# VisualComputingInstitute/diffusion-e2e-ft

Hardware: AMD Instinct MI355X
Metric: images/sec (768x768, 1-step UNet fwd) full path: VAE encode + SD-v2 UNet @t=999 + VAE decode (higher is better)
Workload: dtype f16

## Files before the change

### diffusion-e2e-ft_amd/_lib.py

```python
import ctypes as C
import os

import torch

from . import build as _build

_LIB = None

F32, F16, BF16 = 0, 1, 2
_DT = {torch.float32: F32, torch.float16: F16, torch.bfloat16: BF16}


def dtype_id(dt):
    try:
        return _DT[dt]
    except KeyError:
        raise TypeError("libe2eft supports float32/float16/bfloat16, got %s" % dt)


class ConvDesc(C.Structure):
    _fields_ = [(n, C.c_int32) for n in (
        "dtype", "batch", "hin", "win", "hl", "wl", "c1", "ldx1", "c2", "ldx2", "kh", "kw", "stride", "pad_t", "pad_l",
        "hout", "wout", "cout", "ldo", "ldr", "ldw")] + [("alpha", C.c_float)]

# ... 14 lines not shown
                                          "ldo")] + [("scale", C.c_float)]


class NormalEvalDesc(C.Structure):
    _fields_ = [(n, C.c_int32) for n in ("batch", "height", "width", "reserved")] + [
        ("pred_stride", C.c_int64 * 4), ("gt_stride", C.c_int64 * 4), ("mask_stride", C.c_int64 * 3)]


class D2ntDesc(C.Structure):
    _fields_ = [(n, C.c_int32) for n in ("batch", "height", "width", "refine", "out_format")] + [("depth_scale", C.c_float)]


D2NT_F32, D2NT_U16, D2NT_U8 = range(3)


class HypersimDesc(C.Structure):
    _fields_ = [(n, C.c_int32) for n in ("batch", "height", "width", "color_dtype", "distance_dtype", "depth_format")] + [
        ("focal", C.c_double), ("scale_numerator", C.c_double)]


HYPERSIM_DEPTH_U16, HYPERSIM_DEPTH_F32 = range(2)
HYPERSIM_RECORD = 16


class DepthGtDesc(C.Structure):
    _fields_ = ([(n, C.c_int32) for n in ("batch", "h0", "w0", "raw_dtype")] + [("divisor", C.c_double)]
                + [(n, C.c_int32) for n in ("inf_to_zero", "crop_top", "crop_left", "crop_h", "crop_w")] + [("min_depth", C.c_float), ("max_depth", C.c_float)]
                + [(n, C.c_int32) for n in ("win_y0", "win_y1", "win_x0", "win_x1", "use_ext_mask")])


GT_U16, GT_I32, GT_F32 = range(3)


OPT_PERSISTENT, OPT_PERSISTENT_GRID, OPT_NARROW_CONV, OPT_NARROW_MFMA, OPT_IGEMM_GENERAL_OPERANDS, OPT_IGEMM2_WAVES, OPT_PATCH_CONV, OPT_THIN_INPUT_CONV, OPT_FUSED_NORM, OPT_ATTN_DMA, OPT_UPCONV_PHASES, OPT_PATCH_CONV_2X2, OPT_PERSISTENT_MIN_QROUNDS, OPT_GN_APPLY_ITERS, OPT_F32_SPLIT = range(15)

_P = C.c_void_p
_I = C.c_int32
_L = C.c_int64
_F = C.c_float
_Z = C.c_size_t

SIGNATURES = {
    "e2eft_version": (_I, []),
    "e2eft_last_error": (C.c_char_p, []),
    "e2eft_build_id": (C.c_char_p, []),
    "e2eft_set_option": (_I, [_I, _I]),
    "e2eft_get_option": (_I, [_I]),
    "e2eft_conv2d_fwd": (_I, [C.POINTER(ConvDesc), _P, _P, _P, _P, _P, _P, _P, _P]),
    "e2eft_gemm": (_I, [C.POINTER(GemmDesc), _P, _P, _P, _P, _P, _P]),
    "e2eft_conv2d_fwd_gnstats": (_I, [C.POINTER(ConvDesc), _P, _P, _P, _P, _P, _P, _P, _P, _Z, C.POINTER(C.c_int32), _P]),
    "e2eft_conv2d_splitk_workspace_bytes": (_Z, [C.POINTER(ConvDesc)]),
    "e2eft_conv2d_fwd_splitk": (_I, [C.POINTER(ConvDesc), _P, _P, _P, _P, _P, _P, _P, _P, _Z, _P]),
    "e2eft_gemm_gnstats": (_I, [C.POINTER(GemmDesc), _P, _P, _P, _P, _P, _I, _P, _Z, C.POINTER(C.c_int32), _P]),
    "e2eft_groupnorm_fwd_pre": (_I, [C.POINTER(GroupNormDesc), _P, _P, _P, _P, _P, _P, _I, _P, _I, _P, _Z, _P]),
    "e2eft_groupnorm_coeff_offset": (_Z, [C.POINTER(GroupNormDesc)]),
    "e2eft_groupnorm_fwd_stats": (_I, [C.POINTER(GroupNormDesc), _P, _P, _P, _P, _I, _P, _I, _P, _Z, _P]),
    "e2eft_conv2d_fwd_normed_supported": (_I, [C.POINTER(ConvDesc)]),
    "e2eft_upconv2x_fwd_supported": (_I, [C.POINTER(ConvDesc)]),
    "e2eft_upconv2x_fwd": (_I, [C.POINTER(ConvDesc), _P, _P, _P, _P, _P, _Z, C.POINTER(C.c_int32), _P]),
    "e2eft_groupnorm_fwd_split": (_I, [C.POINTER(GroupNormDesc), _P, _P, _P, _P, _I, _P, _P, _I, _P, _Z, _P]),
    "e2eft_f32_split_weight": (_I, [_P, _L, _I, _P, _P, _P]),
    "e2eft_f32_split2_cat": (_I, [_P, _I, _I, _P, _I, _I, _L, _P, _I, _P, _P]),
    "e2eft_f32_split2": (_I, [_P, _L, _I, _I, _P, _I, _P, _P]),
    "e2eft_conv2d_fwd_f32split_supported": (_I, [C.POINTER(ConvDesc)]),
    "e2eft_conv2d_fwd_f32split": (_I, [C.POINTER(ConvDesc), _P, _P, _P, _P, _P, _P, _P, _P, _Z, C.POINTER(C.c_int32), _P]),
    "e2eft_upconv2x_fwd_f32split_supported": (_I, [C.POINTER(ConvDesc)]),
    "e2eft_upconv2x_fwd_f32split": (_I, [C.POINTER(ConvDesc), _P, _P, _P, _P, _P, _P, _P, _Z, C.POINTER(C.c_int32), _P]),
    "e2eft_gemm_f32split_supported": (_I, [C.POINTER(GemmDesc)]),
    "e2eft_gemm_f32split": (_I, [C.POINTER(GemmDesc), _P, _P, _P, _P, _P, _P, _P, _P]),
    "e2eft_conv2d_fwd_normed": (_I, [C.POINTER(ConvDesc), _P, _P, _P, _I, _P, _P, _P, _P, _P, _P, _Z, C.POINTER(C.c_int32), _P]),
    "e2eft_groupnorm_workspace_bytes": (_Z, [C.POINTER(GroupNormDesc)]),
    "e2eft_groupnorm_fwd": (_I, [C.POINTER(GroupNormDesc), _P, _P, _P, _P, _P, _P, _Z, _P]),
    "e2eft_layernorm_fwd": (_I, [_I, _L, _I, _I, _I, _F, _P, _P, _P, _P, _P]),
    "e2eft_geglu_fwd": (_I, [_I, _L, _I, _I, _I, _P, _P, _P]),
    "e2eft_softmax_rows": (_I, [_I, _L, _I, _L, _F, _P, _P]),
    "e2eft_softmax_rows_causal": (_I, [_I, _L, _I, _L, _F, _I, _P, _P]),
    "e2eft_attn_fwd": (_I, [C.POINTER(AttnDesc), _P, _P, _P, _P, _P]),
    "e2eft_attn_fwd_lse": (_I, [C.POINTER(AttnDesc), _P, _P, _P, _P, _P, _P]),
    "e2eft_attn512_workspace_bytes": (_Z, [C.POINTER(AttnDesc)]),
    "e2eft_attn512_fwd": (_I, [C.POINTER(AttnDesc), _P, _P, _P, _P, _P, _Z, _P]),
    "e2eft_attn_bwd_workspace_bytes": (_Z, [C.POINTER(AttnDesc)]),
    "e2eft_attn_bwd": (_I, [C.POINTER(AttnDesc), _P, _P, _P, _P, _P, _I, _P, _P, _I, _P, _I, _P, _I, _P, _Z, _P]),
    "e2eft_nchw_to_nhwc": (_I, [_I, _I, _I, _I, _I, _I, _I, _F, _F, _P, _P, _P]),
    "e2eft_nhwc_to_nchw": (_I, [_I, _I, _I, _I, _I, _I, _F, _F, _P, _P, _P]),
    "e2eft_copy_scale": (_I, [_I, _L, _I, _I, _I, _F, _F, _P, _P, _P]),
    "e2eft_add": (_I, [_I, _L, _I, _I, _I, _I, _P, _P, _P, _P]),
    "e2eft_timestep_embedding": (_I, [_I, _I, _I, _P, _P, _P]),
    "e2eft_silu": (_I, [_I, _L, _P, _P, _P]),
    "e2eft_depth_head": (_I, [_I, _I, _L, _I, _I, _P, _P, _P]),
    "e2eft_normal_head": (_I, [_I, _I, _I, _I, _I, _I, _F, _P, _P, _P]),
    "e2eft_ssi_loss_workspace_bytes": (_Z, [_I]),
    "e2eft_ssi_loss_fwd": (_I, [_I, _I, _P, _P, _P, _P, _P, _P, _Z, _P]),
    "e2eft_angular_loss_workspace_bytes": (_Z, [_I]),
    "e2eft_angular_loss_fwd": (_I, [_I, _I, _P, _P, _P, _P, _P, _Z, _P]),
    "e2eft_conv2d_dgrad": (_I, [C.POINTER(ConvDesc), _P, _I, _I, _P, _I, _P, _I, _P]),
    "e2eft_conv2d_wgrad_workspace_bytes": (_Z, [C.POINTER(ConvDesc), _I]),
    "e2eft_conv2d_wgrad": (_I, [C.POINTER(ConvDesc), _P, _I, _P, _P, _P, _Z, C.POINTER(C.c_int32), _P]),
    "e2eft_conv2d_im2col_t": (_I, [C.POINTER(ConvDesc), _P, _P, _P, _L, _P]),
    "e2eft_transpose": (_I, [_I, _I, _L, _I, _L, _L, _L, _L, _L, _P, _P, _P]),
    "e2eft_colsum_workspace_bytes": (_Z, [_I, _L, _I]),
    "e2eft_colsum": (_I, [_I, _I, _L, _I, _L, _F, _P, _P, _P, _Z, _P]),
    "e2eft_upsample_nearest_bwd": (_I, [_I, _I, _I, _I, _I, _I, _I, _I, _I, _P, _P, _P]),
    "e2eft_groupnorm_bwd_workspace_bytes": (_Z, [C.POINTER(GroupNormDesc)]),
    "e2eft_groupnorm_bwd": (_I, [C.POINTER(GroupNormDesc), _P, _P, _P, _P, _P, _I, _P, _I, _P, _P, _P, _P, _Z, _P]),
    "e2eft_groupnorm_bwd_add": (_I, [C.POINTER(GroupNormDesc), _P, _P, _P, _P, _P, _I, _P, _I, _P, _I, _P, _P, _P, _P, _Z, _P]),
    "e2eft_layernorm_bwd_workspace_bytes": (_Z, [_L, _I]),
# ... 107 lines not shown
```

### diffusion-e2e-ft_amd/csrc/api.hip

```cpp
#include "common.h"
#include <atomic>

namespace e2eft {

static thread_local char g_err[512] = "";

char* err_buf() { return g_err; }

int fail(int code, const char* fmt, ...) {
    va_list ap;
    va_start(ap, fmt);
    vsnprintf(g_err, sizeof(g_err), fmt, ap);
    va_end(ap);
    return code;
}

int check_launch(const char* what) {
    hipError_t e = hipGetLastError();
    if (e != hipSuccess) return fail(E2EFT_ERR_LAUNCH, "%s: launch failed: %s", what, hipGetErrorString(e));
    return E2EFT_OK;
}

static std::atomic<int> g_cus_of_device[64];
int device_cus() {
    int dev = 0;
    if (hipGetDevice(&dev) != hipSuccess || dev < 0 || dev >= 64) return 0;
    int n = g_cus_of_device[dev].load(std::memory_order_relaxed);
    if (n == 0) {
        if (hipDeviceGetAttribute(&n, hipDeviceAttributeMultiprocessorCount, dev) != hipSuccess || n < 8) return 0;
        n &= ~7;
        g_cus_of_device[dev].store(n, std::memory_order_relaxed);
    }
    return n;
}

static thread_local char g_tag[96] = "";
void tag_kernel(const char* fmt, ...) {
    va_list ap;
    va_start(ap, fmt);
    vsnprintf(g_tag, sizeof(g_tag), fmt, ap);
    va_end(ap);
}
const char* last_tag() { return g_tag; }

static std::atomic<int> g_opt[E2EFT_OPT_COUNT] = {{1}, {0}, {1}, {1}, {0}, {0}, {1}, {1}, {1}, {1}, {1}, {1}, {2}, {0}, {1}};

int option(int key) { return g_opt[key].load(std::memory_order_relaxed); }

}

extern "C" int e2eft_set_option(int32_t key, int32_t value) {
    using namespace e2eft;
    E2EFT_REQUIRE(key >= 0 && key < E2EFT_OPT_COUNT, "set_option: unknown key %d", key);
    bool ok = value == 0 || value == 1;
    if (key == E2EFT_OPT_PERSISTENT_GRID) ok = value == 0 || (value >= 8 && value % 8 == 0 && value <= 4096);
    if (key == E2EFT_OPT_IGEMM2_WAVES) ok = value == 0 || value == 4 || value == 8;
    if (key == E2EFT_OPT_PERSISTENT_MIN_QROUNDS) ok = value >= 1 && value <= 64;
    if (key == E2EFT_OPT_GN_APPLY_ITERS) ok = value >= 0 && value <= 16;
    E2EFT_REQUIRE(ok, "set_option: value %d out of range for key %d", value, key);
    g_opt[key].store(value, std::memory_order_relaxed);
    return E2EFT_OK;
}
extern "C" int e2eft_get_option(int32_t key) { return key >= 0 && key < E2EFT_OPT_COUNT ? e2eft::option(key) : -1; }

extern "C" const char* e2eft_debug_last_kernel(void) { return e2eft::last_tag(); }

extern "C" int e2eft_version(void) { return E2EFT_VERSION; }
#ifndef E2EFT_BUILD_ID
#define E2EFT_BUILD_ID "unstamped"
#endif
static const char k_build_id[] = "E2EFT_BUILD_ID=" E2EFT_BUILD_ID;
extern "C" const char* e2eft_build_id(void) { return k_build_id + 15; }
extern "C" const char* e2eft_last_error(void) { return e2eft::err_buf(); }
```

### diffusion-e2e-ft_amd/csrc/norm.hip

```cpp
#include "common.h"

namespace e2eft {

struct Triple {
    float n, mean, m2;
};
__device__ __forceinline__ Triple merge(const Triple& A, const Triple& B) {
    if (B.n == 0.f) return A;
    if (A.n == 0.f) return B;
    Triple r;
    r.n = A.n + B.n;
    const float delta = B.mean - A.mean;
    const float f = B.n / r.n;
    r.mean = A.mean + delta * f;
    r.m2 = A.m2 + B.m2 + delta * delta * A.n * f;
    return r;
}

struct GnGeom {
    int batch, hw, c1, ldx1, c2, ldx2, C;
    int nchunks, cpb, nchb, pl;
    int nslabs, slab;
};

// ... 552 lines not shown
        const int ch = lane + 64 * i;
        if (ch < nchunks) {
            Vec16<T> t = ld16(x + row * ldx + ch * EPC);
#pragma unroll
            for (int e = 0; e < EPC; ++e) { v[i][e] = to_f(t.e[e]); sum += v[i][e]; }
        } else {
#pragma unroll
            for (int e = 0; e < EPC; ++e) v[i][e] = 0.f;
        }
    }
    const float mean = wave_sum(sum) / (float)c;
    float sq = 0.f;
#pragma unroll
    for (int i = 0; i < MAXI; ++i) {
        const int ch = lane + 64 * i;
        if (ch < nchunks) {
#pragma unroll
            for (int e = 0; e < EPC; ++e) { const float dd = v[i][e] - mean; sq += dd * dd; }
        }
    }
    const float rstd = rsqrtf(wave_sum(sq) / (float)c + eps);
#pragma unroll
    for (int i = 0; i < MAXI; ++i) {
        const int ch = lane + 64 * i;
        if (ch < nchunks) {
            Vec16<T> ga = ld16(gamma + ch * EPC), be = ld16(beta + ch * EPC), o;
#pragma unroll
            for (int e = 0; e < EPC; ++e) o.e[e] = from_f<T>((v[i][e] - mean) * rstd * to_f(ga.e[e]) + to_f(be.e[e]));
            st16(y + row * ldy + ch * EPC, o);
        }
    }
}

template <typename T>
__global__ __launch_bounds__(256) void softmax_rows_kernel(int ntot, long lds, float scale, T* __restrict__ s, int causal_nq) {
    constexpr int EPC = 16 / (int)sizeof(T);
    __shared__ float red[8];
    T* row = s + (long)blockIdx.x * lds;
    const int tid = threadIdx.x, lane = tid & 63, wave = tid >> 6;
    const int n = causal_nq > 0 ? min(ntot, (int)(blockIdx.x % (unsigned)causal_nq) + 1) : ntot;
    const int nfull = n / EPC;
    const float sc = scale * 1.4426950408889634f;
    float mx = -INFINITY;
    for (int ch = tid; ch < nfull; ch += 256) {
        Vec16<T> v = ld16(row + ch * EPC);
#pragma unroll
        for (int e = 0; e < EPC; ++e) mx = fmaxf(mx, to_f(v.e[e]));
    }
    for (int j = nfull * EPC + tid; j < n; j += 256) mx = fmaxf(mx, to_f(row[j]));
    mx = wave_max(mx);
    if (lane == 0) red[wave] = mx;
    __syncthreads();
    mx = fmaxf(fmaxf(red[0], red[1]), fmaxf(red[2], red[3]));
    const float mb = mx * sc;
    float sum = 0.f;
    for (int ch = tid; ch < nfull; ch += 256) {
        Vec16<T> v = ld16(row + ch * EPC);
#pragma unroll
        for (int e = 0; e < EPC; ++e) sum += exp2f(fmaf(to_f(v.e[e]), sc, -mb));
    }
    for (int j = nfull * EPC + tid; j < n; j += 256) sum += exp2f(fmaf(to_f(row[j]), sc, -mb));
    sum = wave_sum(sum);
    if (lane == 0) red[4 + wave] = sum;
    __syncthreads();
    const float inv = 1.f / (red[4] + red[5] + red[6] + red[7]);
    for (int ch = tid; ch < nfull; ch += 256) {
// ... 238 lines not shown
    const int it = option(E2EFT_OPT_GN_APPLY_ITERS);
    g.slab = g.pl * 4 * (it > 0 ? it : (tensor_bytes <= (128L << 20) ? 4 : 2));
    g.nslabs = (d->hw + g.slab - 1) / g.slab;
    hipLaunchKernelGGL(gn_apply_split_kernel, dim3(g.nslabs, g.batch, g.nchb), dim3(256), 0, (hipStream_t)stream, g, d->silu, (int)ldp, (const float*)scale, x, ad, beta, (f16*)planes);
    return check_launch("groupnorm_fwd_split");
}

extern "C" int e2eft_groupnorm_fwd(const E2eftGroupNormDesc* d, const void* x1, const void* x2, const void* gamma,
                                   const void* beta, void* y, void* workspace, size_t ws_bytes, void* stream) {
    return e2eft_groupnorm_fwd_pre(d, x1, x2, gamma, beta, y, nullptr, 0, nullptr, 0, workspace, ws_bytes, stream);
}

extern "C" int e2eft_layernorm_fwd(int32_t dtype, int64_t rows, int32_t c, int32_t ldx, int32_t ldy, float eps,
                                   const void* x, const void* gamma, const void* beta, void* y, void* stream) {
    E2EFT_REQUIRE(x && gamma && beta && y, "layernorm: null pointer");
    E2EFT_REQUIRE(dtype >= 0 && dtype <= 2, "layernorm: bad dtype");
    const int epc = 16 / (int)dtype_size(dtype);
    E2EFT_REQUIRE(rows > 0 && c > 0 && c % epc == 0 && ldx >= c && ldy >= c && ldx % epc == 0 && ldy % epc == 0, "layernorm: shape c=%d ldx=%d ldy=%d", c, ldx, ldy);
    const int nchunks = c / epc;
    E2EFT_REQUIRE(nchunks <= 64 * 8, "layernorm: c=%d too large", c);
    const long nblk = (rows + 3) / 4;
    E2EFT_REQUIRE(nblk < 2147483647L, "layernorm: too many rows");
    hipStream_t s = (hipStream_t)stream;
    const int iters = (nchunks + 63) / 64;
#define LN_LAUNCH(T, MAXI) hipLaunchKernelGGL((layernorm_kernel<T, MAXI>), dim3((unsigned)nblk), dim3(256), 0, s, (long)rows, c, ldx, ldy, eps, (const T*)x, (const T*)gamma, (const T*)beta, (T*)y)
    E2EFT_DISPATCH_DTYPE(dtype, T, {
        if (iters <= 1) LN_LAUNCH(T, 1);
        else if (iters <= 2) LN_LAUNCH(T, 2);
        else if (iters <= 4) LN_LAUNCH(T, 4);
        else LN_LAUNCH(T, 8);
    });
#undef LN_LAUNCH
    return check_launch("layernorm");
}

extern "C" int e2eft_softmax_rows(int32_t dtype, int64_t rows, int32_t n, int64_t lds, float scale, void* sbuf, void* stream) {
    E2EFT_REQUIRE(sbuf, "softmax: null pointer");
    E2EFT_REQUIRE(dtype >= 0 && dtype <= 2, "softmax: bad dtype");
    const int epc = 16 / (int)dtype_size(dtype);
    E2EFT_REQUIRE(rows > 0 && rows < 2147483647L && n > 0 && lds >= (n + epc - 1) / epc * epc && lds % epc == 0, "softmax: shape n=%d lds=%ld", n, (long)lds);
    E2EFT_REQUIRE(scale > 0.f, "softmax: scale must be positive");
    hipStream_t s = (hipStream_t)stream;
    E2EFT_DISPATCH_DTYPE(dtype, T, hipLaunchKernelGGL((softmax_rows_kernel<T>), dim3((unsigned)rows), dim3(256), 0, s, n, (long)lds, scale, (T*)sbuf, 0));
    return check_launch("softmax_rows");
}

extern "C" int e2eft_softmax_rows_causal(int32_t dtype, int64_t rows, int32_t n, int64_t lds, float scale, int32_t nq, void* sbuf, void* stream) {
    E2EFT_REQUIRE(sbuf, "softmax_causal: null pointer");
    E2EFT_REQUIRE(dtype >= 0 && dtype <= 2, "softmax_causal: bad dtype");
    const int epc = 16 / (int)dtype_size(dtype);
    E2EFT_REQUIRE(rows > 0 && rows < 2147483647L && n > 0 && lds >= (n + epc - 1) / epc * epc && lds % epc == 0, "softmax_causal: shape n=%d lds=%ld", n, (long)lds);
    E2EFT_REQUIRE(nq > 0 && nq <= n && rows % nq == 0, "softmax_causal: nq=%d must divide rows and be <= n (self-attention)", nq);
    E2EFT_REQUIRE(scale > 0.f, "softmax_causal: scale must be positive");
    hipStream_t s = (hipStream_t)stream;
    E2EFT_DISPATCH_DTYPE(dtype, T, hipLaunchKernelGGL((softmax_rows_kernel<T>), dim3((unsigned)rows), dim3(256), 0, s, n, (long)lds, scale, (T*)sbuf, (int)nq));
    return check_launch("softmax_rows_causal");
}

extern "C" int e2eft_geglu_fwd(int32_t dtype, int64_t rows, int32_t c, int32_t ldh, int32_t ldy, const void* h, void* y, void* stream) {
    E2EFT_REQUIRE(h && y, "geglu: null pointer");
    E2EFT_REQUIRE(dtype >= 0 && dtype <= 2, "geglu: bad dtype");
    const int epc = 16 / (int)dtype_size(dtype);
    E2EFT_REQUIRE(rows > 0 && c > 0 && c % epc == 0 && ldh >= 2 * c && ldh % epc == 0 && ldy >= c && ldy % epc == 0, "geglu: shape");
    const long total = rows * (c / epc);
    long nb = (total + 255) / 256;
    if (nb > 8192) nb = 8192;
// ... 109 lines not shown
```

### diffusion-e2e-ft_amd/modules.py

```python

import torch
from torch import nn

from . import ops
from . import autograd as F


_cached = F.cached


def packed_conv_weight(conv):
    return F.packed_conv_weight(conv, conv.weight.dtype)


def conv_nhwc(conv, x, x2=None, up_to=None, rowadd=None, residual=None, alpha=1.0, pad=None, out=None, gn_stats=True, norm=None):
    assert out is None
    return F.conv(conv, x, x2=x2, up_to=up_to, rowadd=rowadd, residual=residual, alpha=alpha, pad=pad, gn_stats=gn_stats, norm=norm)


def checkpointed(enabled, fn, *args):
    if enabled and torch.is_grad_enabled() and any(isinstance(a, torch.Tensor) and a.requires_grad for a in args):
        from torch.utils.checkpoint import checkpoint
        return checkpoint(fn, *args, use_reentrant=False)
    return fn(*args)
# ... 167 lines not shown
    ops.softmax_rows_(s.view(-1, nkp), nkt, scale)
    o = torch.empty((B, N, C), dtype=dt, device=dev)
    for qh in range(nseg):
        ops.bgemm_raw(dt, N, d, nkp, s[qh * Bv:], nkp, (heads * N * nkp, N * nkp), vt, nkp, (C * nkp, d * nkp), o[qh * Bv:], C, (N * C, d),
                      Bv, heads)
    return o


class Attention(nn.Module):

    def __init__(self, query_dim, heads, cross_attention_dim=None, bias=False, joint=False):
        super().__init__()
        self.heads = heads
        self.scale = (query_dim // heads) ** -0.5
        self.joint = joint
        kv = cross_attention_dim or query_dim
        self.to_q = Linear(query_dim, query_dim, bias=bias)
        self.to_k = Linear(kv, query_dim, bias=bias)
        self.to_v = Linear(kv, query_dim, bias=bias)
        self.to_out = nn.ModuleList([Linear(query_dim, query_dim), nn.Dropout(0.0)])

    def forward(self, x, ctx=None, residual=None):
        B, N, C = x.shape
        d = C // self.heads
        out = self.to_out[0]
        kv_pre = None
        shared_src = None
        if isinstance(ctx, CtxCond):
            kv_pre = ctx.kv.get(id(self))
            shared_src = ctx.src if ctx.shared else None
            ctx = ctx.ctx
        if F.needs_grad(x, ctx, self.to_q.weight, self.to_k.weight, self.to_v.weight, out.weight):
            return out(self._forward_train(x, ctx), residual=residual)
        if (CROSS_ATTN_FOLD and shared_src is not None and shared_src.shape[1] == 2 and not self.joint and self.to_q.bias is None and self.to_k.bias is None
                and self.to_v.bias is None and self.heads <= 64):
            return self._folded(x, shared_src, residual)
        fused = F.fused_attention_ok(x.dtype, d)
        dt = x.dtype
        if fused:
            if ctx is None:
                qkv = F.linear(x, (self.to_q.weight, self.to_k.weight, self.to_v.weight), owner=self, name="wqkv")
                q, k, v = qkv[..., :C], qkv[..., C:2 * C], qkv[..., 2 * C:]
            else:
                q = self.to_q(x)
                kv = kv_pre
                if kv is None or torch.is_grad_enabled():
                    kv = F.linear(ctx, (self.to_k.weight, self.to_v.weight), owner=self, name="wkv")
                k, v = kv[..., :C], kv[..., C:]
            a = ops.attention(q, k, v, self.heads, self.scale, kv_nseg=2 if self.joint else 1, kv_bmod=B // 2 if self.joint else B)
        else:
            src = x if ctx is None else ctx
            cw = lambda lin: F._cat_weight(lin, "w", (lin.weight,), dt, lin.weight.shape[1])
            a = attention_unfused(x, src, cw(self.to_q), F._vec(self.to_q.bias, dt), cw(self.to_k), F._vec(self.to_k.bias, dt), cw(self.to_v),
                                  F._vec(self.to_v.bias, dt), self.heads, self.scale, joint=self.joint)
        return out(a, residual=residual)

    def _fold(self, src, dt):
        out = self.to_out[0]
        ws = [w for w in (self.to_q.weight, self.to_k.weight, self.to_v.weight, out.weight, out.bias) if w is not None]
        key = (src.data_ptr(), src._version, tuple(src.shape), str(src.device), dt, F._key(*ws))
        hit = self.__dict__.get("_fold_cache")
        if hit is not None and hit[0] == key:
            return hit[1]
        with torch.no_grad():
            h, C = self.heads, self.to_q.weight.shape[0]
            d = C // h
            f32 = lambda w: w.detach().float().contiguous()
            wq, wk, wv, wo = f32(self.to_q.weight), f32(self.to_k.weight), f32(self.to_v.weight), f32(out.weight)
            c32 = f32(src[0])
            k = ops.gemm(c32, wk)
            v = ops.gemm(c32, wv)
            ar = torch.arange(h, device=k.device)
            Mk = torch.zeros((h, h, d), dtype=torch.float32, device=k.device)
            Mv = torch.zeros((h, h, d), dtype=torch.float32, device=k.device)
            Mk[ar, ar] = (k[0] - k[1]).view(h, d) * self.scale
            Mv[ar, ar] = (v[0] - v[1]).view(h, d)
            G = ops.gemm(Mk.view(h, C), wq.t().contiguous())
            delta = ops.gemm(Mv.view(h, C), wo)
            c0 = ops.gemm(v[1:2].contiguous(), wo, f32(out.bias) if out.bias is not None else None)[0]
            hp = ops.round_up(h, ops.epc(dt))
            Gp = torch.zeros((hp, C), dtype=torch.float32, device=G.device)
            Gp[:h] = G
            Dt = torch.zeros((C, hp), dtype=torch.float32, device=G.device)
            Dt[:, :h] = delta.t()
            val = (Gp.to(dt).contiguous(), Dt.to(dt).contiguous(), c0.to(dt).contiguous())
        self.__dict__["_fold_cache"] = (key, val, src)
        return val

# ... 22 lines not shown
class GEGLU(nn.Module):

    def __init__(self, dim, inner):
        super().__init__()
        self.proj = Linear(dim, 2 * inner)

    def forward(self, x):
        return F.geglu(self.proj(x))


class FeedForward(nn.Module):

    def __init__(self, dim):
        super().__init__()
        self.net = nn.ModuleList([GEGLU(dim, 4 * dim), nn.Dropout(0.0), Linear(4 * dim, dim)])

    def forward(self, x, residual=None):
        return self.net[2](self.net[0](x), residual=residual)


class BasicTransformerBlock(nn.Module):

    def __init__(self, dim, heads, cross_attention_dim, joint=False):
        super().__init__()
        self.norm1 = LayerNorm(dim, eps=1e-5)
        self.attn1 = Attention(dim, heads, joint=joint)
        self.norm2 = LayerNorm(dim, eps=1e-5)
        self.attn2 = Attention(dim, heads, cross_attention_dim=cross_attention_dim)
        self.norm3 = LayerNorm(dim, eps=1e-5)
        self.ff = FeedForward(dim)

    def forward(self, h, ctx):
        h = self.attn1(self.norm1(h), None, residual=h)
        h = self.attn2(self.norm2(h), ctx, residual=h)
        return self.ff(self.norm3(h), residual=h)


class Transformer2DModel(nn.Module):

    def __init__(self, channels, heads, cross_attention_dim, groups=32, joint=False):
        super().__init__()
        self.norm = GroupNorm(groups, channels, eps=1e-6, affine=True)
        self.proj_in = Linear(channels, channels)
        self.transformer_blocks = nn.ModuleList([BasicTransformerBlock(channels, heads, cross_attention_dim, joint=joint)])
        self.proj_out = Linear(channels, channels)

    def nhwc(self, x, ctx):
        B, H, W, C = x.shape
        h, x = self.norm.nhwc(x, split=True)
        h = self.proj_in(h.view(B, H * W, C))
        for blk in self.transformer_blocks:
            h = blk(h, ctx)
        out = self.proj_out(h, residual=x.reshape(B, H * W, C), gn_rows_per_image=H * W)
        res = out.view(B, H, W, C)
        st = getattr(out, "_e2eft_gn", None)
        if st is not None:
            res._e2eft_gn = st
        return res


class VaeAttention(nn.Module):

    def __init__(self, channels, groups=32):
        super().__init__()
        self.group_norm = GroupNorm(groups, channels, eps=1e-6, affine=True)
        self.to_q = Linear(channels, channels)
        self.to_k = Linear(channels, channels)
        self.to_v = Linear(channels, channels)
# ... 28 lines not shown
```

### diffusion-e2e-ft_amd/ops.py

```python
import ctypes as C

import torch

from . import _lib
from ._lib import ConvDesc, GemmDesc, GroupNormDesc, AttnDesc, check, dtype_id


class KernelTimer:

    def __init__(self, only=None):
        self.rec = {}
        self.only = only

    def add(self, name, start, end, flops, nbytes, label=None, launches=1, flops_nominal=None):
        self.rec.setdefault(name, []).append((start, end, flops, nbytes, label, launches, flops if flops_nominal is None else flops_nominal))

    def summary(self):
        torch.cuda.synchronize()
        out = {}
        for name, lst in self.rec.items():
            ms = sum(r[0].elapsed_time(r[1]) for r in lst)
            out[name] = dict(launches=sum(r[5] for r in lst), ms=ms, flops=float(sum(r[2] for r in lst)), bytes=float(sum(r[3] for r in lst)),
                             flops_nominal=float(sum(r[6] for r in lst)))
        return out
# ... 570 lines not shown
def groupnorm_stats(x, gamma, groups, eps):
    _check_cuda(x, gamma)
    B, H, W, c1 = x.shape
    d = GroupNormDesc()
    d.dtype = dtype_id(x.dtype)
    d.batch, d.hw = B, H * W
    d.c1, d.ldx1, d.c2, d.ldx2 = c1, _nhwc_ld(x), 0, 0
    d.groups, d.ldy, d.silu, d.eps = groups, c1, 0, eps
    lib = _lib.load()
    nbytes = lib.e2eft_groupnorm_workspace_bytes(C.byref(d))
    if nbytes == 0:
        raise RuntimeError("groupnorm_stats: %s" % lib.e2eft_last_error().decode())
    ws = torch.empty((nbytes + 3) // 4, dtype=torch.float32, device=x.device)
    s1 = getattr(x, "_e2eft_gn", None) if GN_STATS_ENABLED else None
    with _timed("groupnorm_stats", 0.0, 0.0, label="gn stats B%d %dx%d C%d" % (B, H, W, c1)):
        check(lib.e2eft_groupnorm_fwd_stats(C.byref(d), _ptr(x), C.c_void_p(0), _ptr(gamma), _ptr(s1.partial) if s1 else C.c_void_p(0), s1.nslabs if s1 else 0,
                                            C.c_void_p(0), 0, _ptr(ws), nbytes, _stream()))
    return ws, ws.data_ptr() + lib.e2eft_groupnorm_coeff_offset(C.byref(d))


def layernorm(x, gamma, beta, eps, out=None):
    _check_cuda(x, gamma, beta, out)
    Cc = x.shape[-1]
    a = x.reshape(-1, Cc) if x.is_contiguous() else _as_rows(x)
    if out is None:
        out = torch.empty(x.shape, dtype=x.dtype, device=x.device)
    o = out.reshape(-1, Cc) if out.is_contiguous() else _as_rows(out)
    assert gamma.dtype == x.dtype and beta.dtype == x.dtype
    check(_lib.load().e2eft_layernorm_fwd(dtype_id(x.dtype), a.shape[0], Cc, _rows_ld(a), _rows_ld(o), eps, _ptr(a), _ptr(gamma),
                                         _ptr(beta), _ptr(o), _stream()))
    return out


def geglu(h, out=None):
    _check_cuda(h, out)
    c2 = h.shape[-1]
    c = c2 // 2
    a = h.reshape(-1, c2) if h.is_contiguous() else _as_rows(h)
    if out is None:
        out = torch.empty((*h.shape[:-1], c), dtype=h.dtype, device=h.device)
    o = out.reshape(-1, c) if out.is_contiguous() else _as_rows(out)
    check(_lib.load().e2eft_geglu_fwd(dtype_id(h.dtype), a.shape[0], c, _rows_ld(a), _rows_ld(o), _ptr(a), _ptr(o), _stream()))
    return out


def softmax_rows_(s, n, scale, causal_nq=0):
    _check_cuda(s)
    assert s.dim() == 2 and s.is_contiguous()
    if causal_nq:
        check(_lib.load().e2eft_softmax_rows_causal(dtype_id(s.dtype), s.shape[0], n, s.shape[1], scale, causal_nq, _ptr(s), _stream()))
    else:
        check(_lib.load().e2eft_softmax_rows(dtype_id(s.dtype), s.shape[0], n, s.shape[1], scale, _ptr(s), _stream()))
    return s


def _ld3(t):
    if t.shape[2] > 1 and t.stride(2) != 1:
        raise ValueError("attention operands need unit inner stride")
    ld = t.stride(1) if t.shape[1] > 1 else max(t.shape[2], t.stride(1))
    if t.shape[0] > 1 and t.stride(0) != t.shape[1] * ld:
        raise ValueError("attention operands must be batch-dense: %s %s" % (tuple(t.shape), t.stride()))
    return ld


def _attn_desc(q, k, v, out, heads, scale, kv_nseg, kv_bmod):
    B, Nq, Wd = q.shape
# ... 907 lines not shown
```

### include/e2eft.h

```cpp
#ifndef E2EFT_H
#define E2EFT_H

#include <stddef.h>
#include <stdint.h>

#ifdef __cplusplus
extern "C" {
#endif
#pragma GCC visibility push(default)

#define E2EFT_VERSION 119

enum {
    E2EFT_OK = 0,
    E2EFT_ERR_BAD_ARG = 1,
    E2EFT_ERR_WORKSPACE = 2,
    E2EFT_ERR_LAUNCH = 3,
    E2EFT_ERR_UNSUPPORTED = 4,
};

enum { E2EFT_F32 = 0, E2EFT_F16 = 1, E2EFT_BF16 = 2 };

int e2eft_version(void);
const char* e2eft_last_error(void);
const char* e2eft_build_id(void);

enum {
    E2EFT_OPT_PERSISTENT = 0,
    E2EFT_OPT_PERSISTENT_GRID = 1,
    E2EFT_OPT_NARROW_CONV = 2,
    E2EFT_OPT_NARROW_MFMA = 3,
    E2EFT_OPT_IGEMM_GENERAL_OPERANDS = 4,
    E2EFT_OPT_IGEMM2_WAVES = 5,
    E2EFT_OPT_PATCH_CONV = 6,
    E2EFT_OPT_THIN_INPUT_CONV = 7,
    E2EFT_OPT_FUSED_NORM = 8,
    E2EFT_OPT_ATTN_DMA = 9,
    E2EFT_OPT_UPCONV_PHASES = 10,
    E2EFT_OPT_PATCH_CONV_2X2 = 11,
    E2EFT_OPT_PERSISTENT_MIN_QROUNDS = 12,
    E2EFT_OPT_GN_APPLY_ITERS = 13,
    E2EFT_OPT_F32_SPLIT = 14,
    E2EFT_OPT_COUNT = 15
};
int e2eft_set_option(int32_t key, int32_t value);
int e2eft_get_option(int32_t key);

typedef struct E2eftConvDesc {
    int32_t dtype;
    int32_t batch, hin, win, hl, wl;
    int32_t c1, ldx1;
    int32_t c2, ldx2;
    int32_t kh, kw, stride;
    int32_t pad_t, pad_l;
    int32_t hout, wout;
    int32_t cout, ldo;
    int32_t ldr;
    int32_t ldw;
    float alpha;
} E2eftConvDesc;

int e2eft_conv2d_fwd(const E2eftConvDesc* d, const void* x1, const void* x2, const void* w,
                     const void* bias ,
                     const void* rowadd ,
                     const void* residual , void* out, void* stream);

typedef struct E2eftGemmDesc {
    int32_t dtype;
    int32_t m, n, k;
    int32_t lda, ldw, ldo, ldr;
    int32_t nzo, nzi;
    int64_t sa_o, sa_i, sw_o, sw_i, so_o, so_i, sr_o, sr_i;
    int32_t bias_along_m;
    float alpha;
} E2eftGemmDesc;

// ... 27 lines not shown
size_t e2eft_conv2d_splitk_workspace_bytes(const E2eftConvDesc* d);
int e2eft_conv2d_fwd_splitk(const E2eftConvDesc* d, const void* x1, const void* x2, const void* w, const void* bias,
                            const void* rowadd, const void* residual, void* out, void* workspace, size_t ws_bytes, void* stream);
int e2eft_gemm_gnstats(const E2eftGemmDesc* d, const void* a, const void* w, const void* bias, const void* residual,
                       void* out, int32_t rows_per_image, float* gn_partial, size_t gn_partial_bytes,
                       int32_t* slab_rows, void* stream);

typedef struct E2eftGroupNormDesc {
    int32_t dtype;
    int32_t batch, hw;
    int32_t c1, ldx1, c2, ldx2;
    int32_t groups;
    int32_t ldy;
    int32_t silu;
    float eps;
} E2eftGroupNormDesc;

size_t e2eft_groupnorm_workspace_bytes(const E2eftGroupNormDesc* d);
int e2eft_groupnorm_fwd(const E2eftGroupNormDesc* d, const void* x1, const void* x2, const void* gamma,
                        const void* beta, void* y, void* workspace, size_t ws_bytes, void* stream);

int e2eft_groupnorm_fwd_split(const E2eftGroupNormDesc* d, const float* x, const float* gamma, const float* beta, void* planes, int32_t ldp, float* scale,
                              const float* partial1, int32_t nslabs1, void* workspace, size_t ws_bytes, void* stream);

int e2eft_groupnorm_fwd_pre(const E2eftGroupNormDesc* d, const void* x1, const void* x2, const void* gamma,
                            const void* beta, void* y, const float* partial1, int32_t nslabs1, const float* partial2,
                            int32_t nslabs2, void* workspace, size_t ws_bytes, void* stream);
size_t e2eft_groupnorm_coeff_offset(const E2eftGroupNormDesc* d);
int e2eft_groupnorm_fwd_stats(const E2eftGroupNormDesc* d, const void* x1, const void* x2, const void* gamma, const float* partial1,
                              int32_t nslabs1, const float* partial2, int32_t nslabs2, void* workspace, size_t ws_bytes, void* stream);

int e2eft_layernorm_fwd(int32_t dtype, int64_t rows, int32_t c, int32_t ldx, int32_t ldy, float eps,
                        const void* x, const void* gamma, const void* beta, void* y, void* stream);

int e2eft_geglu_fwd(int32_t dtype, int64_t rows, int32_t c, int32_t ldh, int32_t ldy, const void* h, void* y,
                    void* stream);

int e2eft_softmax_rows(int32_t dtype, int64_t rows, int32_t n, int64_t lds, float scale, void* s, void* stream);
int e2eft_softmax_rows_causal(int32_t dtype, int64_t rows, int32_t n, int64_t lds, float scale, int32_t nq, void* s, void* stream);

typedef struct E2eftAttnDesc {
    int32_t dtype;
    int32_t batch, heads, nq, nk_seg;
    int32_t kv_nseg, kv_bmod;
    int32_t ldq, ldk, ldv, ldo;
    float scale;
} E2eftAttnDesc;

int e2eft_attn_fwd(const E2eftAttnDesc* d, const void* q, const void* k, const void* v, void* out, void* stream);
int e2eft_attn_fwd_lse(const E2eftAttnDesc* d, const void* q, const void* k, const void* v, void* out, float* lse, void* stream);
size_t e2eft_attn512_workspace_bytes(const E2eftAttnDesc* d);
int e2eft_attn512_fwd(const E2eftAttnDesc* d, const void* q, const void* k, const void* v, void* out, void* workspace, size_t ws_bytes,
                      void* stream);
size_t e2eft_conv2d_wgrad_workspace_bytes(const E2eftConvDesc* d, int32_t lddy);
int e2eft_conv2d_wgrad(const E2eftConvDesc* d, const void* dy, int32_t lddy, const void* x1, const void* x2, float* partial, size_t partial_bytes,
                       int32_t* nsplit_out, void* stream);
size_t e2eft_attn_bwd_workspace_bytes(const E2eftAttnDesc* d);
int e2eft_attn_bwd(const E2eftAttnDesc* d, const void* q, const void* k, const void* v, const void* out, const void* dout,
                   int32_t lddo, const float* lse, void* dq, int32_t lddq, void* dk, int32_t lddk, void* dv, int32_t lddv,
                   void* workspace, size_t ws_bytes, void* stream);


int e2eft_nchw_to_nhwc(int32_t dt_in, int32_t dt_out, int32_t batch, int32_t c, int32_t hw, int32_t cpad,
                       int32_t ldy, float mul, float add, const void* x, void* y, void* stream);
int e2eft_nhwc_to_nchw(int32_t dt_in, int32_t dt_out, int32_t batch, int32_t c, int32_t hw, int32_t ldx,
                       float mul, float add, const void* x, void* y, void* stream);
// ... 149 lines not shown
```

Before: 91.68.

## Fuse LayerNorm2, folded cross-attention, residual and LayerNorm3 into one kernel

Adds a single kernel that performs norm2, the folded two-token cross-attention (a G projection, a sigmoid blend, then a Dt projection), the residual add and norm3 per row, with G, Dt and the norm parameters staged in shared memory. The transformer block calls it when the cross-attention fold applies, replacing several separate launches and intermediate tensor round trips through global memory. The cost is a large LDS footprint and scalar FMA dot products in place of MFMA. It adds intermediate fp16 roundings that are meant to match the unfused path.

```diff
diff --git a/diffusion-e2e-ft_amd/_lib.py b/diffusion-e2e-ft_amd/_lib.py
--- a/diffusion-e2e-ft_amd/_lib.py
+++ b/diffusion-e2e-ft_amd/_lib.py
@@ -70,7 +70,7 @@
 GT_U16, GT_I32, GT_F32 = range(3)
 
 
-OPT_PERSISTENT, OPT_PERSISTENT_GRID, OPT_NARROW_CONV, OPT_NARROW_MFMA, OPT_IGEMM_GENERAL_OPERANDS, OPT_IGEMM2_WAVES, OPT_PATCH_CONV, OPT_THIN_INPUT_CONV, OPT_FUSED_NORM, OPT_ATTN_DMA, OPT_UPCONV_PHASES, OPT_PATCH_CONV_2X2, OPT_PERSISTENT_MIN_QROUNDS, OPT_GN_APPLY_ITERS, OPT_F32_SPLIT = range(15)
+OPT_PERSISTENT, OPT_PERSISTENT_GRID, OPT_NARROW_CONV, OPT_NARROW_MFMA, OPT_IGEMM_GENERAL_OPERANDS, OPT_IGEMM2_WAVES, OPT_PATCH_CONV, OPT_THIN_INPUT_CONV, OPT_FUSED_NORM, OPT_ATTN_DMA, OPT_UPCONV_PHASES, OPT_PATCH_CONV_2X2, OPT_PERSISTENT_MIN_QROUNDS, OPT_GN_APPLY_ITERS, OPT_F32_SPLIT, OPT_FUSED_CROSS_FOLD = range(16)
 
 _P = C.c_void_p
 _I = C.c_int32
@@ -110,6 +110,7 @@
     "e2eft_groupnorm_workspace_bytes": (_Z, [C.POINTER(GroupNormDesc)]),
     "e2eft_groupnorm_fwd": (_I, [C.POINTER(GroupNormDesc), _P, _P, _P, _P, _P, _P, _Z, _P]),
     "e2eft_layernorm_fwd": (_I, [_I, _L, _I, _I, _I, _F, _P, _P, _P, _P, _P]),
+    "e2eft_cross_fold_ln_fwd": (_I, [_I, _L, _I, _I, _P, _P, _P, _P, _P, _P, _P, _P, _F, _P, _P, _P]),
     "e2eft_geglu_fwd": (_I, [_I, _L, _I, _I, _I, _P, _P, _P]),
     "e2eft_softmax_rows": (_I, [_I, _L, _I, _L, _F, _P, _P]),
     "e2eft_softmax_rows_causal": (_I, [_I, _L, _I, _L, _F, _I, _P, _P]),
diff --git a/diffusion-e2e-ft_amd/csrc/api.hip b/diffusion-e2e-ft_amd/csrc/api.hip
--- a/diffusion-e2e-ft_amd/csrc/api.hip
+++ b/diffusion-e2e-ft_amd/csrc/api.hip
@@ -43,7 +43,7 @@
 }
 const char* last_tag() { return g_tag; }
 
-static std::atomic<int> g_opt[E2EFT_OPT_COUNT] = {{1}, {0}, {1}, {1}, {0}, {0}, {1}, {1}, {1}, {1}, {1}, {1}, {2}, {0}, {1}};
+static std::atomic<int> g_opt[E2EFT_OPT_COUNT] = {{1}, {0}, {1}, {1}, {0}, {0}, {1}, {1}, {1}, {1}, {1}, {1}, {2}, {0}, {1}, {1}};
 
 int option(int key) { return g_opt[key].load(std::memory_order_relaxed); }
 
diff --git a/diffusion-e2e-ft_amd/csrc/norm.hip b/diffusion-e2e-ft_amd/csrc/norm.hip
--- a/diffusion-e2e-ft_amd/csrc/norm.hip
+++ b/diffusion-e2e-ft_amd/csrc/norm.hip
@@ -608,6 +608,166 @@
     }
 }
 
+template <typename T, int MAXI>
+__global__ __launch_bounds__(512) void cross_fold_ln_kernel(long rows, int c, int hp, float eps, const T* __restrict__ x, const T* __restrict__ g2,
+                                                            const T* __restrict__ b2, const T* __restrict__ G, const T* __restrict__ Dt,
+                                                            const T* __restrict__ c0, const T* __restrict__ g3, const T* __restrict__ b3,
+                                                            T* __restrict__ out_x, T* __restrict__ out_ln3) {
+    constexpr int EPC = 8;
+    static_assert(sizeof(T) == 2, "16-bit rows");
+    __shared__ __attribute__((aligned(16))) T lds[2 * 8 * MAXI * 512 * MAXI + 5 * 512 * MAXI];
+    T* sG = lds;
+    T* sD = lds + hp * c;
+    T* sP = sD + hp * c;
+    const int tid = threadIdx.x, lane = tid & 63, wave = tid >> 6;
+    const int nchunks = c / EPC;
+    for (int it = tid; it < hp * nchunks; it += 512) *reinterpret_cast<u32x4*>(sG + it * EPC) = *reinterpret_cast<const u32x4*>(G + it * EPC);
+    for (int it = tid; it < hp * c; it += 512) {
+        const int col = it / hp, hh = it - col * hp;
+        sD[hh * c + col] = Dt[it];
+    }
+    for (int it = tid; it < 5 * nchunks; it += 512) {
+        const int which = it / nchunks, ch = it - which * nchunks;
+        const T* src = which == 0 ? g2 : which == 1 ? b2 : which == 2 ? c0 : which == 3 ? g3 : b3;
+        *reinterpret_cast<u32x4*>(sP + it * EPC) = *reinterpret_cast<const u32x4*>(src + ch * EPC);
+    }
+    __syncthreads();
+    const long stride = (long)gridDim.x * 8;
+    long row = (long)blockIdx.x * 8 + wave;
+    if (row >= rows) return;
+    bool act[MAXI];
+    int cofs[MAXI];
+    Vec16<T> cur[MAXI], nxt[MAXI];
+#pragma unroll
+    for (int i = 0; i < MAXI; ++i) {
+        const int ch = lane + 64 * i;
+        act[i] = ch < nchunks;
+        cofs[i] = act[i] ? ch * EPC : 0;
+        cur[i] = ld16(x + row * c + cofs[i]);
+    }
+    const bool k32 = (lane & 32) != 0, k16 = (lane & 16) != 0, k8 = (lane & 8) != 0;
+    for (; row < rows; row += stride) {
+        const long rnext = row + stride < rows ? row + stride : row;
+#pragma unroll
+        for (int i = 0; i < MAXI; ++i) nxt[i] = ld16(x + rnext * c + cofs[i]);
+        float v[MAXI][EPC];
+        float sum = 0.f;
+#pragma unroll
+        for (int i = 0; i < MAXI; ++i) {
+            if (act[i]) {
+#pragma unroll
+                for (int e = 0; e < EPC; ++e) { v[i][e] = to_f(cur[i].e[e]); sum += v[i][e]; }
+            } else {
+#pragma unroll
+                for (int e = 0; e < EPC; ++e) v[i][e] = 0.f;
+            }
+        }
+        float mean = wave_sum(sum) / (float)c;
+        float sq = 0.f;
+#pragma unroll
+        for (int i = 0; i < MAXI; ++i) {
+            if (act[i]) {
+#pragma unroll
+                for (int e = 0; e < EPC; ++e) { const float dd = v[i][e] - mean; sq += dd * dd; }
+            }
+        }
+        float rstd = rsqrtf(wave_sum(sq) / (float)c + eps);
+        float nrm[MAXI][EPC], acc[MAXI][EPC];
+#pragma unroll
+        for (int i = 0; i < MAXI; ++i) {
+            const Vec16<T> ga = ld16(sP + cofs[i]), be = ld16(sP + c + cofs[i]);
+#pragma unroll
+            for (int e = 0; e < EPC; ++e) {
+                nrm[i][e] = act[i] ? to_f(from_f<T>((v[i][e] - mean) * rstd * to_f(ga.e[e]) + to_f(be.e[e]))) : 0.f;
+                acc[i][e] = 0.f;
+            }
+        }
+        for (int h0 = 0; h0 < hp; h0 += 8) {
+            float d[8];
+#pragma unroll
+            for (int k = 0; k < 8; ++k) {
+                float s = 0.f;
+#pragma unroll
+                for (int i = 0; i < MAXI; ++i) {
+                    const Vec16<T> gv = ld16(sG + (h0 + k) * c + cofs[i]);
+#pragma unroll
+                    for (int e = 0; e < EPC; ++e) s = fmaf(nrm[i][e], to_f(gv.e[e]), s);
+                }
+                d[k] = s;
+                if (k & 1) __builtin_amdgcn_sched_barrier(0);
+            }
+#pragma unroll
+            for (int k = 0; k < 4; ++k) {
+                const float keep = k32 ? d[k + 4] : d[k], send = k32 ? d[k] : d[k + 4];
+                d[k] = keep + __shfl_xor(send, 32, 64);
+            }
+#pragma unroll
+            for (int k = 0; k < 2; ++k) {
+                const float keep = k16 ? d[k + 2] : d[k], send = k16 ? d[k] : d[k + 2];
+                d[k] = keep + __shfl_xor(send, 16, 64);
+            }
+            {
+                const float keep = k8 ? d[1] : d[0], send = k8 ? d[0] : d[1];
+                d[0] = keep + __shfl_xor(send, 8, 64);
+            }
+            float t = d[0];
+            t += __shfl_xor(t, 4, 64);
+            t += __shfl_xor(t, 2, 64);
+            t += __shfl_xor(t, 1, 64);
+            const float sg = to_f(from_f<T>(t));
+            const float pl = to_f(from_f<T>(__builtin_amdgcn_rcpf(1.0f + __expf(-sg))));
+#pragma unroll
+            for (int k = 0; k < 8; ++k) {
+                const float pk = __int_as_float(__builtin_amdgcn_readlane(__float_as_int(pl), ((k >> 2) & 1) * 32 + ((k >> 1) & 1) * 16 + (k & 1) * 8));
+#pragma unroll
+                for (int i = 0; i < MAXI; ++i) {
+                    const Vec16<T> dv = ld16(sD + (h0 + k) * c + cofs[i]);
+#pragma unroll
+                    for (int e = 0; e < EPC; ++e) acc[i][e] = fmaf(pk, to_f(dv.e[e]), acc[i][e]);
+                }
+                if (k & 1) __builtin_amdgcn_sched_barrier(0);
+            }
+        }
+        sum = 0.f;
+#pragma unroll
+        for (int i = 0; i < MAXI; ++i) {
+            const Vec16<T> cv = ld16(sP + 2 * c + cofs[i]);
+            Vec16<T> o;
+#pragma unroll
+            for (int e = 0; e < EPC; ++e) {
+                o.e[e] = from_f<T>((acc[i][e] + to_f(cv.e[e])) + v[i][e]);
+                v[i][e] = act[i] ? to_f(o.e[e]) : 0.f;
+            }
+            if (act[i]) {
+                st16(out_x + row * c + cofs[i], o);
+#pragma unroll
+                for (int e = 0; e < EPC; ++e) sum += v[i][e];
+            }
+        }
+        mean = wave_sum(sum) / (float)c;
+        sq = 0.f;
+#pragma unroll
+        for (int i = 0; i < MAXI; ++i) {
+            if (act[i]) {
+#pragma unroll
+                for (int e = 0; e < EPC; ++e) { const float dd = v[i][e] - mean; sq += dd * dd; }
+            }
+        }
+        rstd = rsqrtf(wave_sum(sq) / (float)c + eps);
+#pragma unroll
+        for (int i = 0; i < MAXI; ++i) {
+            if (act[i]) {
+                const Vec16<T> ga = ld16(sP + 3 * c + cofs[i]), be = ld16(sP + 4 * c + cofs[i]);
+                Vec16<T> o;
+#pragma unroll
+                for (int e = 0; e < EPC; ++e) o.e[e] = from_f<T>((v[i][e] - mean) * rstd * to_f(ga.e[e]) + to_f(be.e[e]));
+                st16(out_ln3 + row * c + cofs[i], o);
+            }
+            cur[i] = nxt[i];
+        }
+    }
+}
+
 template <typename T>
 __global__ __launch_bounds__(256) void softmax_rows_kernel(int ntot, long lds, float scale, T* __restrict__ s, int causal_nq) {
     constexpr int EPC = 16 / (int)sizeof(T);
@@ -912,6 +1072,36 @@
     });
 #undef LN_LAUNCH
     return check_launch("layernorm");
+}
+
+extern "C" int e2eft_cross_fold_ln_fwd(int32_t dtype, int64_t rows, int32_t c, int32_t hp, const void* x, const void* ln2_gamma, const void* ln2_beta,
+                                       const void* G, const void* Dt, const void* c0, const void* ln3_gamma, const void* ln3_beta, float eps,
+                                       void* out_x, void* out_ln3, void* stream) {
+    E2EFT_REQUIRE(x && ln2_gamma && ln2_beta && G && Dt && c0 && ln3_gamma && ln3_beta && out_x && out_ln3, "cross_fold_ln: null pointer");
+    E2EFT_REQUIRE(dtype >= 0 && dtype <= 2, "cross_fold_ln: bad dtype");
+    E2EFT_REQUIRE(rows > 0 && c > 0 && hp > 0, "cross_fold_ln: shape rows=%ld c=%d hp=%d", (long)rows, c, hp);
+    if (!option(E2EFT_OPT_FUSED_CROSS_FOLD)) return fail(E2EFT_ERR_UNSUPPORTED, "cross_fold_ln: switched off (E2EFT_OPT_FUSED_CROSS_FOLD = 0)");
+    if (dtype == E2EFT_F32 || c % 8 != 0 || hp % 8 != 0 || c > 1536 || hp > 24)
+        return fail(E2EFT_ERR_UNSUPPORTED, "cross_fold_ln: 16-bit rows of c <= 1536 (a multiple of 8) and hp <= 24 (a multiple of 8); got dtype %d c=%d hp=%d", dtype, c, hp);
+    E2EFT_REQUIRE(al16(x) && al16(ln2_gamma) && al16(ln2_beta) && al16(G) && al16(c0) && al16(ln3_gamma) && al16(ln3_beta) && al16(out_x) && al16(out_ln3),
+                  "cross_fold_ln: buffers must be 16-byte aligned");
+    const int cus = device_cus();
+    if (cus <= 0) return fail(E2EFT_ERR_LAUNCH, "cross_fold_ln: no device");
+    int maxi = (c / 8 + 63) / 64;
+    if (hp > 8 * maxi) maxi = hp / 8;
+    const long want = (rows + 7) / 8, cap = (long)cus * (maxi == 1 ? 2 : 1);
+    const unsigned nblk = (unsigned)(want < cap ? want : cap);
+    hipStream_t s = (hipStream_t)stream;
+#define CF_LAUNCH(T, MAXI) hipLaunchKernelGGL((cross_fold_ln_kernel<T, MAXI>), dim3(nblk), dim3(512), 0, s, (long)rows, c, hp, eps, (const T*)x, (const T*)ln2_gamma, \
+        (const T*)ln2_beta, (const T*)G, (const T*)Dt, (const T*)c0, (const T*)ln3_gamma, (const T*)ln3_beta, (T*)out_x, (T*)out_ln3)
+    if (dtype == E2EFT_F16) {
+        if (maxi == 1) CF_LAUNCH(f16, 1); else if (maxi == 2) CF_LAUNCH(f16, 2); else CF_LAUNCH(f16, 3);
+    } else {
+        if (maxi == 1) CF_LAUNCH(bf16, 1); else if (maxi == 2) CF_LAUNCH(bf16, 2); else CF_LAUNCH(bf16, 3);
+    }
+#undef CF_LAUNCH
+    tag_kernel("cross_fold_ln_kernel<%s, %d>", dtype == E2EFT_F16 ? "_Float16" : "__bf16", maxi);
+    return check_launch("cross_fold_ln");
 }
 
 extern "C" int e2eft_softmax_rows(int32_t dtype, int64_t rows, int32_t n, int64_t lds, float scale, void* sbuf, void* stream) {
diff --git a/diffusion-e2e-ft_amd/modules.py b/diffusion-e2e-ft_amd/modules.py
--- a/diffusion-e2e-ft_amd/modules.py
+++ b/diffusion-e2e-ft_amd/modules.py
@@ -223,8 +223,7 @@
             ctx = ctx.ctx
         if F.needs_grad(x, ctx, self.to_q.weight, self.to_k.weight, self.to_v.weight, out.weight):
             return out(self._forward_train(x, ctx), residual=residual)
-        if (CROSS_ATTN_FOLD and shared_src is not None and shared_src.shape[1] == 2 and not self.joint and self.to_q.bias is None and self.to_k.bias is None
-                and self.to_v.bias is None and self.heads <= 64):
+        if self._foldable(shared_src):
             return self._folded(x, shared_src, residual)
         fused = F.fused_attention_ok(x.dtype, d)
         dt = x.dtype
@@ -245,6 +244,18 @@
             a = attention_unfused(x, src, cw(self.to_q), F._vec(self.to_q.bias, dt), cw(self.to_k), F._vec(self.to_k.bias, dt), cw(self.to_v),
                                   F._vec(self.to_v.bias, dt), self.heads, self.scale, joint=self.joint)
         return out(a, residual=residual)
+
+    def _foldable(self, shared_src):
+        return (CROSS_ATTN_FOLD and shared_src is not None and shared_src.shape[1] == 2 and not self.joint and self.to_q.bias is None and self.to_k.bias is None
+                and self.to_v.bias is None and self.heads <= 64)
+
+    def fold_operands(self, x, ctx):
+        if not isinstance(ctx, CtxCond) or not ctx.shared or not self._foldable(ctx.src):
+            return None
+        out = self.to_out[0]
+        if F.needs_grad(x, ctx.ctx, self.to_q.weight, self.to_k.weight, self.to_v.weight, out.weight):
+            return None
+        return self._fold(ctx.src, x.dtype)
 
     def _fold(self, src, dt):
         out = self.to_out[0]
@@ -333,8 +344,23 @@
 
     def forward(self, h, ctx):
         h = self.attn1(self.norm1(h), None, residual=h)
+        fused = self._cross_fold_ln(h, ctx)
+        if fused is not None:
+            h, n3 = fused
+            return self.ff(n3, residual=h)
         h = self.attn2(self.norm2(h), ctx, residual=h)
         return self.ff(self.norm3(h), residual=h)
+
+    def _cross_fold_ln(self, h, ctx):
+        n2, n3 = self.norm2, self.norm3
+        if h.dtype == torch.float32 or n2.eps != n3.eps or not h.is_contiguous() or F.needs_grad(h, n2.weight, n2.bias, n3.weight, n3.bias):
+            return None
+        fold = self.attn2.fold_operands(h, ctx)
+        if fold is None:
+            return None
+        dt = h.dtype
+        with ops.on_device_of(h):
+            return ops.cross_fold_ln(h, F._vec(n2.weight, dt), F._vec(n2.bias, dt), *fold, F._vec(n3.weight, dt), F._vec(n3.bias, dt), n2.eps)
 
 
 class Transformer2DModel(nn.Module):
diff --git a/diffusion-e2e-ft_amd/ops.py b/diffusion-e2e-ft_amd/ops.py
--- a/diffusion-e2e-ft_amd/ops.py
+++ b/diffusion-e2e-ft_amd/ops.py
@@ -626,6 +626,21 @@
     return out
 
 
+def cross_fold_ln(x, ln2_gamma, ln2_beta, G, Dt, c0, ln3_gamma, ln3_beta, eps):
+    _check_cuda(x, ln2_gamma, ln2_beta, G, Dt, c0, ln3_gamma, ln3_beta)
+    Cc, hp = x.shape[-1], G.shape[0]
+    assert x.is_contiguous() and G.is_contiguous() and Dt.is_contiguous() and G.shape == (hp, Cc) and Dt.shape == (Cc, hp) and c0.shape == (Cc,)
+    assert all(t.dtype == x.dtype for t in (ln2_gamma, ln2_beta, G, Dt, c0, ln3_gamma, ln3_beta))
+    lib = _lib.load()
+    out_x, out_n = torch.empty_like(x), torch.empty_like(x)
+    rc = lib.e2eft_cross_fold_ln_fwd(dtype_id(x.dtype), x.numel() // Cc, Cc, hp, _ptr(x), _ptr(ln2_gamma), _ptr(ln2_beta), _ptr(G), _ptr(Dt), _ptr(c0),
+                                     _ptr(ln3_gamma), _ptr(ln3_beta), eps, _ptr(out_x), _ptr(out_n), _stream())
+    if rc == 4:
+        return None
+    check(rc)
+    return out_x, out_n
+
+
 def geglu(h, out=None):
     _check_cuda(h, out)
     c2 = h.shape[-1]
diff --git a/include/e2eft.h b/include/e2eft.h
--- a/include/e2eft.h
+++ b/include/e2eft.h
@@ -41,7 +41,8 @@
     E2EFT_OPT_PERSISTENT_MIN_QROUNDS = 12,
     E2EFT_OPT_GN_APPLY_ITERS = 13,
     E2EFT_OPT_F32_SPLIT = 14,
-    E2EFT_OPT_COUNT = 15
+    E2EFT_OPT_FUSED_CROSS_FOLD = 15,
+    E2EFT_OPT_COUNT = 16
 };
 int e2eft_set_option(int32_t key, int32_t value);
 int e2eft_get_option(int32_t key);
@@ -135,6 +136,10 @@
 
 int e2eft_layernorm_fwd(int32_t dtype, int64_t rows, int32_t c, int32_t ldx, int32_t ldy, float eps,
                         const void* x, const void* gamma, const void* beta, void* y, void* stream);
+
+int e2eft_cross_fold_ln_fwd(int32_t dtype, int64_t rows, int32_t c, int32_t hp, const void* x, const void* ln2_gamma, const void* ln2_beta,
+                            const void* G, const void* Dt, const void* c0, const void* ln3_gamma, const void* ln3_beta, float eps,
+                            void* out_x, void* out_ln3, void* stream);
 
 int e2eft_geglu_fwd(int32_t dtype, int64_t rows, int32_t c, int32_t ldh, int32_t ldy, const void* h, void* y,
                     void* stream);
```

Result: no change. 91.95, median of 6 (+0.3%).
